# Coder-Yu/QRec

Hardware: NVIDIA H100
Metric: BPR triples/sec at d=64 (higher is better)
Workload: dtype f32

## Files before the change

### qrec_b200/csrc/bpr_kernels.cu

```cuda
#include <cmath>

#include "common.h"
#include "device.cuh"
#include "lane_shape.h"
#include "philox.cuh"
#include "bpr_step.cuh"
#include "um_waves.cuh"

namespace {

using namespace qrec;
using namespace qrec::bpr;

template <typename T, int E>
__global__ void __launch_bounds__(256)
bpr_sgd_ordered_kernel(T* __restrict__ P, T* __restrict__ Q, int d, long long n,
                       const int* __restrict__ u, const int* __restrict__ i,
                       const int* __restrict__ j, const int* __restrict__ wu,
                       const int* __restrict__ wi, const int* __restrict__ wj, int* ver_p,
                       int* ver_q, unsigned long long* ticket, T lr, T reg_u, T reg_i,
                       double* loss) {
  const int lane = threadIdx.x & 31;
  double local_loss = 0.0;
  const T a_u = mul_rn(lr, reg_u), a_i = mul_rn(lr, reg_i);
  while (true) {
    unsigned long long k = 0;
    if (lane == 0) k = atomicAdd(ticket, 1ULL);
    k = __shfl_sync(0xffffffffu, k, 0);
    if (k >= (unsigned long long)n) break;
    const int uu = u[k], ii = i[k], jj = j[k];
    const int* vp = lane == 0 ? ver_p + uu : (lane == 1 ? ver_q + ii : ver_q + jj);
    const int need = lane == 0 ? wu[k] : (lane == 1 ? wi[k] : wj[k]);
    unsigned backoff = 8, polls = 0;
    while (true) {
      const int have = lane < 3 ? ld_acquire_gpu(vp) : need;
      if (__all_sync(0xffffffffu, have == need)) break;
      __nanosleep(backoff);
      if (backoff < 64) backoff <<= 1;
      if (++polls > (1u << 27)) __trap();
    }
    T* pr = P + (size_t)uu * d;
    T* qir = Q + (size_t)ii * d;
    T* qjr = Q + (size_t)jj * d;
    T p[E], qi[E], qj[E];
    T di = 0, dj = 0;
#pragma unroll
    for (int e = 0; e < E; ++e) {
      const int c = e * 32 + lane;
      if (c < d) {
        p[e] = __ldcg(pr + c);
        qi[e] = __ldcg(qir + c);
        qj[e] = __ldcg(qjr + c);
        di += p[e] * qi[e];
        dj += p[e] * qj[e];
      } else {
        p[e] = qi[e] = qj[e] = 0;
      }
    }
    di = warp_sum(di);
    dj = warp_sum(dj);
    const T s = sigmoid_full(sub_rn(di, dj));
    const T g = mul_rn(lr, sub_rn((T)1, s));
#pragma unroll
    for (int e = 0; e < E; ++e) {
      const int c = e * 32 + lane;
      if (c < d) {
        T pn, qin, qjn;
        bpr_update_parity(p[e], qi[e], qj[e], g, a_u, a_i, pn, qin, qjn);
        __stcg(pr + c, pn);
        __stcg(qir + c, qin);
        __stcg(qjr + c, qjn);
      }
    }
    __threadfence();
    __syncwarp();
    if (lane < 3) red_release_gpu_add(const_cast<int*>(vp), 1);
    if (lane == 0) local_loss += neg_log(s);
  }
  if (lane == 0 && local_loss != 0.0) atomicAdd(loss, local_loss);
}

template <int LPR, int VPL, int UNROLL>
__global__ void __launch_bounds__(256)
bpr_sgd_batch_kernel(float* __restrict__ P, float* __restrict__ Q, int nvec, long long n,
                     const int* __restrict__ u, const int* __restrict__ i,
                     const int* __restrict__ j, float lr, float reg_u, float reg_i,
                     double* loss) {
  constexpr int TPW = 32 / LPR;
  const int lane = threadIdx.x & 31;
  const int sub = lane / LPR, l = lane % LPR;
  const long long warp = ((long long)blockIdx.x * blockDim.x + threadIdx.x) >> 5;
  const long long nwarps = ((long long)gridDim.x * blockDim.x) >> 5;
  const int d = nvec * 4;
  const float a_u = lr * reg_u, a_i = lr * reg_i;
  float lsum = 0.f;

  for (long long base = warp * 32; base < n; base += nwarps * 32) {
    const long long k = base + lane;
    int mu = 0, mi = 0, mj = 0;
    if (k < n) {
      mu = __ldg(u + k);
      mi = __ldg(i + k);
      mj = __ldg(j + k);
    }
    const int cnt = (n - base) < 32 ? (int)(n - base) : 32;
    for (int s0 = 0; s0 < cnt; s0 += TPW * UNROLL) {
      float4 p[UNROLL][VPL], qi[UNROLL][VPL], qj[UNROLL][VPL];
      float* pr[UNROLL];
      float* qir[UNROLL];
      float* qjr[UNROLL];
      bool ok[UNROLL];
#pragma unroll
      for (int r = 0; r < UNROLL; ++r) {
        const int t = s0 + r * TPW + sub;
        const int uu = __shfl_sync(0xffffffffu, mu, t & 31);
        const int ii = __shfl_sync(0xffffffffu, mi, t & 31);
        const int jj = __shfl_sync(0xffffffffu, mj, t & 31);
        ok[r] = t < cnt;
        pr[r] = P + (size_t)uu * d + l * 4;
        qir[r] = Q + (size_t)ii * d + l * 4;
        qjr[r] = Q + (size_t)jj * d + l * 4;
#pragma unroll
        for (int v = 0; v < VPL; ++v) {
          if (ok[r] && (l + v * LPR) < nvec) {
            p[r][v] = *reinterpret_cast<const float4*>(pr[r] + v * LPR * 4);
            qi[r][v] = *reinterpret_cast<const float4*>(qir[r] + v * LPR * 4);
            qj[r][v] = *reinterpret_cast<const float4*>(qjr[r] + v * LPR * 4);
          } else {
            p[r][v] = qi[r][v] = qj[r][v] = make_float4(0.f, 0.f, 0.f, 0.f);
          }
        }
      }
#pragma unroll
      for (int r = 0; r < UNROLL; ++r) {
        float x = 0.f;
#pragma unroll
        for (int v = 0; v < VPL; ++v) x += dot4(p[r][v], qi[r][v]) - dot4(p[r][v], qj[r][v]);
        x = group_sum<LPR>(x);
        const float s = fast_sigmoid(x);
        const float g = lr * (1.0f - s);
        if (ok[r]) {
          if (l == 0) lsum += fast_neg_log(s);
#pragma unroll
          for (int v = 0; v < VPL; ++v) {
            if ((l + v * LPR) < nvec) {
              float4 dp, dqi, dqj;
              bpr_step4(p[r][v], qi[r][v], qj[r][v], g, a_u, a_i, dp, dqi, dqj);
              red_add_v4(pr[r] + v * LPR * 4, dp);
              red_add_v4(qir[r] + v * LPR * 4, dqi);
              red_add_v4(qjr[r] + v * LPR * 4, dqj);
            }
          }
        }
      }
    }
  }
  block_add_loss(lsum, loss);
}


template <int LPR>
__global__ void __launch_bounds__(256)
bpr_sgd_staged_kernel(float* __restrict__ P, int nvec, long long n, const int* __restrict__ u,
                      const int* __restrict__ pos_i, const int* __restrict__ pos_j,
                      const float* __restrict__ R, float* __restrict__ D, float lr, float reg_u,
                      float reg_i, double* loss) {
  constexpr int TPW = 32 / LPR;
  const int lane = threadIdx.x & 31;
  const int sub = lane / LPR, l = lane % LPR;
  const long long group = (((long long)blockIdx.x * blockDim.x + threadIdx.x) >> 5) * TPW + sub;
  const long long ngroups = (((long long)gridDim.x * blockDim.x) >> 5) * TPW;
  const int d = nvec * 4;
  const float a_u = lr * reg_u, a_i = lr * reg_i;
  float lsum = 0.f;
  const long long rounds = (n + ngroups - 1) / ngroups;
  for (long long it = 0; it < rounds; ++it) {
    const long long k = it * ngroups + group;
    const bool ok = k < n && l < nvec;
    float4 p = make_float4(0.f, 0.f, 0.f, 0.f), qi = p, qj = p;
    float* pr = nullptr;
    size_t oi = 0, oj = 0;
    if (ok) {
      pr = P + (size_t)__ldg(u + k) * d + l * 4;
      oi = (size_t)__ldg(pos_i + k) * d + l * 4;
      oj = (size_t)__ldg(pos_j + k) * d + l * 4;
      p = *reinterpret_cast<const float4*>(pr);
      qi = __ldg(reinterpret_cast<const float4*>(R + oi));
      qj = __ldg(reinterpret_cast<const float4*>(R + oj));
    }
    float x = dot4(p, qi) - dot4(p, qj);
    x = group_sum<LPR>(x);
    const float s = fast_sigmoid(x);
    const float g = lr * (1.0f - s);
    if (ok) {
      if (l == 0) lsum += fast_neg_log(s);
      float4 dp, dqi, dqj;
      bpr_step4(p, qi, qj, g, a_u, a_i, dp, dqi, dqj);
      red_add_v4(pr, dp);
      *reinterpret_cast<float4*>(D + oi) = dqi;
      *reinterpret_cast<float4*>(D + oj) = dqj;
    }
  }
  block_add_loss(lsum, loss);
}


template <int UNROLL, int TMA_MASK>
__global__ void __launch_bounds__(256)
bpr_sgd_batch_tma_kernel(float* __restrict__ P, float* __restrict__ Q, long long n,
                         const int* __restrict__ u, const int* __restrict__ i,
                         const int* __restrict__ j, float lr, float reg_u, float reg_i,
                         double* loss) {
  constexpr int LPR = 16, TPW = 2, D = 64;
  constexpr int ROWS = ((TMA_MASK >> 0) & 1) + ((TMA_MASK >> 1) & 1) + ((TMA_MASK >> 2) & 1);
  constexpr int SLOT_P = 0, SLOT_I = (TMA_MASK & 1), SLOT_J = (TMA_MASK & 1) + ((TMA_MASK >> 1) & 1);
  constexpr int SLOT_FLOATS = UNROLL * TPW * ROWS * D;
  extern __shared__ __align__(128) float stage[];
  const int lane = threadIdx.x & 31, wib = threadIdx.x >> 5;
  const int sub = lane / LPR, l = lane % LPR;
  const long long warp = ((long long)blockIdx.x * blockDim.x + threadIdx.x) >> 5;
  const long long nwarps = ((long long)gridDim.x * blockDim.x) >> 5;
  const float a_u = lr * reg_u, a_i = lr * reg_i;
  float* my_stage = stage + (size_t)wib * 2 * SLOT_FLOATS;
  float lsum = 0.f;
  int buf = 0;

  for (long long base = warp * 32; base < n; base += nwarps * 32) {
    const long long k = base + lane;
    int mu = 0, mi = 0, mj = 0;
    if (k < n) {
      mu = __ldg(u + k);
      mi = __ldg(i + k);
      mj = __ldg(j + k);
    }
    const int cnt = (n - base) < 32 ? (int)(n - base) : 32;
    for (int s0 = 0; s0 < cnt; s0 += TPW * UNROLL) {
      float4 p[UNROLL], qi[UNROLL], qj[UNROLL];
      int uu[UNROLL], ii[UNROLL], jj[UNROLL];
      bool ok[UNROLL];
#pragma unroll
      for (int r = 0; r < UNROLL; ++r) {
        const int t = s0 + r * TPW + sub;
        uu[r] = __shfl_sync(0xffffffffu, mu, t & 31);
        ii[r] = __shfl_sync(0xffffffffu, mi, t & 31);
        jj[r] = __shfl_sync(0xffffffffu, mj, t & 31);
        ok[r] = t < cnt;
        if (ok[r]) {
          p[r] = *reinterpret_cast<const float4*>(P + (size_t)uu[r] * D + l * 4);
          qi[r] = *reinterpret_cast<const float4*>(Q + (size_t)ii[r] * D + l * 4);
          qj[r] = *reinterpret_cast<const float4*>(Q + (size_t)jj[r] * D + l * 4);
        } else {
          p[r] = qi[r] = qj[r] = make_float4(0.f, 0.f, 0.f, 0.f);
        }
      }
      if (l < 3) asm volatile("cp.async.bulk.wait_group.read 1;" ::: "memory");
      __syncwarp();
      float* slot = my_stage + (size_t)buf * SLOT_FLOATS;
#pragma unroll
      for (int r = 0; r < UNROLL; ++r) {
        float x = dot4(p[r], qi[r]) - dot4(p[r], qj[r]);
        x = group_sum<LPR>(x);
        const float s = fast_sigmoid(x);
        const float g = lr * (1.0f - s);
        if (ok[r]) {
          if (l == 0) lsum += fast_neg_log(s);
          float4 dp, dqi, dqj;
          bpr_step4(p[r], qi[r], qj[r], g, a_u, a_i, dp, dqi, dqj);
          float* trip = slot + (size_t)(r * TPW + sub) * ROWS * D;
          if (TMA_MASK & 1) *reinterpret_cast<float4*>(trip + SLOT_P * D + l * 4) = dp;
          else red_add_v4(P + (size_t)uu[r] * D + l * 4, dp);
          if (TMA_MASK & 2) *reinterpret_cast<float4*>(trip + SLOT_I * D + l * 4) = dqi;
          else red_add_v4(Q + (size_t)ii[r] * D + l * 4, dqi);
          if (TMA_MASK & 4) *reinterpret_cast<float4*>(trip + SLOT_J * D + l * 4) = dqj;
          else red_add_v4(Q + (size_t)jj[r] * D + l * 4, dqj);
        }
      }
      asm volatile("fence.proxy.async.shared::cta;" ::: "memory");
      __syncwarp();
      if (l < 3 && ((TMA_MASK >> l) & 1)) {
        const int srow = (l == 0) ? SLOT_P : (l == 1 ? SLOT_I : SLOT_J);
#pragma unroll
        for (int r = 0; r < UNROLL; ++r) {
          if (ok[r]) {
            float* dst = (l == 0) ? (P + (size_t)uu[r] * D) : (Q + (size_t)(l == 1 ? ii[r] : jj[r]) * D);
            const float* src = slot + (size_t)(r * TPW + sub) * ROWS * D + srow * D;
            asm volatile("cp.reduce.async.bulk.global.shared::cta.bulk_group.add.f32 [%0], [%1], %2;" ::"l"(dst),
                         "r"((uint32_t)__cvta_generic_to_shared(src)), "n"(D * 4)
                         : "memory");
          }
        }
        asm volatile("cp.async.bulk.commit_group;" ::: "memory");
      }
      buf ^= 1;
    }
  }
  if (l < 3) asm volatile("cp.async.bulk.wait_group 0;" ::: "memory");
  block_add_loss(lsum, loss);
}


template <int LPR, int G, bool FULL, bool SAMPLE, int MINB = 3, bool SIG = false>
__global__ void __launch_bounds__(256, MINB)
bpr_sgd_usermajor_kernel(float* __restrict__ P, float* __restrict__ Q, const float* __restrict__ Qr, int nvec, long long n,
                         const int* __restrict__ wave_user, const long long* __restrict__ rowptr,
                         const int* __restrict__ i, const int* __restrict__ j, float lr, float reg_u, float reg_i,
                         double* loss, FusedSampler fs, long long trip_off, const uint32_t* __restrict__ rated_sig) {
  constexpr int GPW = 32 / LPR;
  const int lane = threadIdx.x & 31;
  const int sub = lane / LPR, l = lane % LPR;
  const unsigned gmask = (LPR == 32) ? 0xffffffffu : (((1u << LPR) - 1u) << (sub * LPR));
  const int group = (int)((blockIdx.x * blockDim.x + threadIdx.x) >> 5) * GPW + sub;
  const int ngroups = (int)((gridDim.x * blockDim.x) >> 5) * GPW;
  const int d = FULL ? LPR * 4 : nvec * 4;
  const bool act = FULL ? true : (l < nvec);
  const float a_u = lr * reg_u, a_i = lr * reg_i;
  const float one_m_au = 1.0f - a_u, one_m_ai = 1.0f - a_i;
  float lsum = 0.f;
  qrec::pdl_launch_dependents();
  bool waited = false;
  const int ub = __ldg(wave_user + 1);
  for (int uu = __ldg(wave_user) + group; uu < ub; uu += ngroups) {
    long long lo = __ldg(rowptr + uu) - trip_off, hi = __ldg(rowptr + uu + 1) - trip_off;
    lo = lo > 0 ? lo : 0;
    hi = hi < n ? hi : n;
    if (lo >= hi) continue;
    float* prow = P + (size_t)uu * d + l * 4;
    float4 p = act ? *reinterpret_cast<const float4*>(prow) : make_float4(0.f, 0.f, 0.f, 0.f);
    long long rated_lo = 0, rated_hi = 0;
    if (SAMPLE) {
      rated_lo = __ldg(fs.rated_rowptr + uu);
      rated_hi = __ldg(fs.rated_rowptr + uu + 1);
    }
    for (long long base = lo; base < hi; base += LPR) {
      const int m = (hi - base) < LPR ? (int)(hi - base) : LPR;
      int mj = 0, mi = 0;
      if (l < m) {
        mi = __ldg(i + base + l);
        if (SAMPLE) {
          if (SIG)
            mj = qrec::sample_negative_sig(base + l + trip_off, fs.epoch, fs.seed_lo, fs.seed_hi, fs.num_items,
                                           fs.rated_cols, rated_lo, rated_hi,
                                           rated_sig + (size_t)uu * qrec::RATED_SIG_WORDS);
          else
            mj = qrec::sample_negative(base + l + trip_off, fs.epoch, fs.seed_lo, fs.seed_hi, fs.num_items, fs.rated_cols,
                                       rated_lo, rated_hi);
        } else {
          mj = __ldg(j + base + l);
        }
      }
      if (!waited) {
        qrec::pdl_wait();
        waited = true;
      }
      if (SAMPLE && l < m && fs.j_out != nullptr) fs.j_out[base + l] = mj;
      for (int t0 = 0; t0 < m; t0 += G) {
        float4 qi[G], qj[G];
        int ri[G], rj[G];
#pragma unroll
        for (int f = 0; f < G; ++f) {
          ri[f] = __shfl_sync(gmask, mi, sub * LPR + ((t0 + f) & (LPR - 1)));
          rj[f] = __shfl_sync(gmask, mj, sub * LPR + ((t0 + f) & (LPR - 1)));
          if (t0 + f < m && act) {
            qi[f] = qrec::ldg_no_l1_v4(reinterpret_cast<const float4*>(Qr + (size_t)ri[f] * d + l * 4));
            qj[f] = qrec::ldg_no_l1_v4(reinterpret_cast<const float4*>(Qr + (size_t)rj[f] * d + l * 4));
          } else {
            qi[f] = qj[f] = make_float4(0.f, 0.f, 0.f, 0.f);
          }
        }
#pragma unroll
        for (int f = 0; f < G; ++f) {
          if (t0 + f < m) {
            float x = dot4(p, qi[f]) - dot4(p, qj[f]);
            x = group_sum<LPR>(x, gmask);
            const float s = fast_sigmoid(x);
            const float g = lr * (1.0f - s);
            if (l == 0) lsum += fast_neg_log(s);
            if (act) {
              float4 dqi, dqj;
              bpr_step4_inplace(p, qi[f], qj[f], g, one_m_au, g * one_m_ai, a_i, dqi, dqj);
              red_add_v4(Q + (size_t)ri[f] * d + l * 4, dqi);
              red_add_v4(Q + (size_t)rj[f] * d + l * 4, dqj);
            }
          }
        }
      }
    }
    if (act) {
      const float4 p0 = __ldcg(reinterpret_cast<const float4*>(prow));
      red_add_v4(prow, make_float4(p.x - p0.x, p.y - p0.y, p.z - p0.z, p.w - p0.w));
    }
  }
  if (!waited) qrec::pdl_wait();
  block_add_loss(lsum, loss);
}

using UserMajorKernel = decltype(&bpr_sgd_usermajor_kernel<16, 4, true, false>);

template <int LPR>
UserMajorKernel usermajor_kernel(int nvec, bool sample, bool sig) {
  if (nvec != LPR)
    return sample ? bpr_sgd_usermajor_kernel<LPR, 4, false, true> : bpr_sgd_usermajor_kernel<LPR, 4, false, false>;
  if (sig) return bpr_sgd_usermajor_kernel<LPR, 2, true, true, 4, true>;
  return sample ? bpr_sgd_usermajor_kernel<LPR, 2, true, true, 4> : bpr_sgd_usermajor_kernel<LPR, 4, true, false>;
}

constexpr int UM_SNAPSHOT_THREADS = 512, UM_SNAPSHOT_CTAS_PER_SM = 4;
__global__ void __launch_bounds__(UM_SNAPSHOT_THREADS, UM_SNAPSHOT_CTAS_PER_SM)
um_snapshot_kernel(const float4* __restrict__ Q, float4* __restrict__ Qr, long long n4) {
  const unsigned long long keep = qrec::l2_policy_evict_last();
  qrec::pdl_wait();
  qrec::pdl_launch_dependents();
  const long long stride = (long long)gridDim.x * blockDim.x;
  long long k = (long long)blockIdx.x * blockDim.x + threadIdx.x;
  for (; k + 3 * stride < n4; k += 4 * stride) {
    float4 v[4];
#pragma unroll
    for (int r = 0; r < 4; ++r) v[r] = qrec::ld_stream_v4(Q + k + r * stride, keep);
#pragma unroll
    for (int r = 0; r < 4; ++r) qrec::st_hint_v4(Qr + k + r * stride, v[r], keep);
  }
  for (; k < n4; k += stride) qrec::st_hint_v4(Qr + k, qrec::ld_stream_v4(Q + k, keep), keep);
}

__global__ void __launch_bounds__(256)
um_wave_table_kernel(const long long* __restrict__ rowptr, int n_users, long long n, long long trip_off,
                     long long wave_chunks, long long nwaves, int* __restrict__ wave_user) {
  const long long w = (long long)blockIdx.x * blockDim.x + threadIdx.x;
  if (w <= nwaves) wave_user[w] = um_wave_first_user(rowptr, n_users, n, trip_off, wave_chunks, w);
}

__global__ void __launch_bounds__(256)
rated_signature_kernel(int n_users, const long long* __restrict__ rowptr, const int* __restrict__ cols,
                       uint32_t* __restrict__ sig) {
  const int lane = threadIdx.x & 31;
  const long long warp = ((long long)blockIdx.x * blockDim.x + threadIdx.x) >> 5;
  const long long nwarps = ((long long)gridDim.x * blockDim.x) >> 5;
  for (long long uu = warp; uu < n_users; uu += nwarps) {
    const long long lo = __ldg(rowptr + uu), hi = __ldg(rowptr + uu + 1);
    for (long long e = lo + lane; e < hi; e += 32) {
      const int c = __ldg(cols + e);
      atomicOr(sig + (size_t)uu * qrec::RATED_SIG_WORDS + ((c >> 5) & (qrec::RATED_SIG_WORDS - 1)), 1u << (c & 31));
    }
  }
}

template <typename T>
__global__ void __launch_bounds__(256)
sumsq_kernel(const T* __restrict__ x, long long n, double* out) {
  double acc = 0.0;
  const long long tid = (long long)blockIdx.x * blockDim.x + threadIdx.x;
  const long long stride = (long long)gridDim.x * blockDim.x;
  if constexpr (sizeof(T) == 4) {
    const long long n4 = n >> 2;
    const float4* x4 = reinterpret_cast<const float4*>(x);
    for (long long k = tid; k < n4; k += stride) {
      const float4 v = __ldg(x4 + k);
      acc += (double)v.x * v.x + (double)v.y * v.y + (double)v.z * v.z + (double)v.w * v.w;
    }
    for (long long k = (n4 << 2) + tid; k < n; k += stride) acc += (double)x[k] * x[k];
  } else {
    for (long long k = tid; k < n; k += stride) acc += (double)x[k] * (double)x[k];
  }
  acc = warp_sum(acc);
  __shared__ double wsum[8];
  if ((threadIdx.x & 31) == 0) wsum[threadIdx.x >> 5] = acc;
  __syncthreads();
  if (threadIdx.x == 0) {
    double t = 0.0;
    for (int w = 0; w < (int)(blockDim.x >> 5); ++w) t += wsum[w];
    atomicAdd(out, t);
  }
}

template <typename T>
int launch_ordered(T* P, T* Q, int d, long long n, const int* u, const int* i, const int* j,
                   const int* wu, const int* wi, const int* wj, int* ver_p, int* ver_q,
                   unsigned long long* ticket, T lr, T reg_u, T reg_i, double* loss,
                   int n_warps, cudaStream_t st) {
  QREC_REQUIRE(P && Q && loss && ticket && ver_p && ver_q, "bpr_sgd_ordered: null pointer");
  QREC_REQUIRE(d >= 1 && d <= 256, "bpr_sgd_ordered: d=%d unsupported (1..256)", d);
  QREC_REQUIRE(n >= 0, "bpr_sgd_ordered: n < 0");
  if (n == 0) return QREC_OK;
  QREC_REQUIRE(u && i && j && wu && wi && wj, "bpr_sgd_ordered: null index pointer");
  const int grid = n_warps > 0 ? capped_grid((n_warps + 7) / 8, 2) : sm_count() * 2;
  with_lane_elems(d, [&](auto e) {
    bpr_sgd_ordered_kernel<T, decltype(e)::E><<<grid, 256, 0, st>>>(P, Q, d, n, u, i, j, wu, wi, wj, ver_p, ver_q,
                                                                    ticket, lr, reg_u, reg_i, loss);
  });
  QREC_LAUNCH_CHECK();
  return QREC_OK;
}

}

namespace qrec {
int launch_bpr_batch(float* P, float* Q, int d, long long n, const int* u, const int* i,
                     const int* j, float lr, float reg_u, float reg_i, double* loss,
                     cudaStream_t st) {
  QREC_REQUIRE(P && Q && loss, "bpr_sgd_batch: null pointer");
  QREC_REQUIRE(d >= 4 && d <= 256 && (d % 4) == 0, "bpr_sgd_batch: d=%d unsupported (multiple of 4, 4..256)", d);
  QREC_REQUIRE(n >= 0, "bpr_sgd_batch: n < 0");
  if (n == 0) return QREC_OK;
  QREC_REQUIRE(u && i && j, "bpr_sgd_batch: null index pointer");
  const int nvec = d / 4;
  const long long warps_needed = (n + 31) / 32;
  const int grid = capped_grid((warps_needed + 7) / 8, 8);
  with_row_shape<256>(nvec, [&](auto s) {
    using S = decltype(s);
    bpr_sgd_batch_kernel<S::LPR, S::VPL, S::UNROLL><<<grid, 256, 0, st>>>(P, Q, nvec, n, u, i, j, lr, reg_u, reg_i,
                                                                          loss);
  });
  QREC_LAUNCH_CHECK();
  return QREC_OK;
}
}

extern "C" {

int qrec_bpr_sgd_ordered_f32(float* P, float* Q, int32_t d, int64_t n, const int32_t* u,
                             const int32_t* i, const int32_t* j, const int32_t* wu,
                             const int32_t* wi, const int32_t* wj, int32_t* ver_p,
                             int32_t* ver_q, unsigned long long* ticket, float lr, float reg_u,
                             float reg_i, double* loss, int32_t n_warps, void* stream) {
  return launch_ordered<float>(P, Q, d, n, u, i, j, wu, wi, wj, ver_p, ver_q, ticket, lr, reg_u,
                               reg_i, loss, n_warps, (cudaStream_t)stream);
}

int qrec_bpr_sgd_ordered_f64(double* P, double* Q, int32_t d, int64_t n, const int32_t* u,
                             const int32_t* i, const int32_t* j, const int32_t* wu,
                             const int32_t* wi, const int32_t* wj, int32_t* ver_p,
                             int32_t* ver_q, unsigned long long* ticket, double lr,
                             double reg_u, double reg_i, double* loss, int32_t n_warps, void* stream) {
  return launch_ordered<double>(P, Q, d, n, u, i, j, wu, wi, wj, ver_p, ver_q, ticket, lr, reg_u,
                                reg_i, loss, n_warps, (cudaStream_t)stream);
}

int qrec_bpr_sgd_batch_f32(float* P, float* Q, int32_t d, int64_t n, const int32_t* u,
                           const int32_t* i, const int32_t* j, float lr, float reg_u,
                           float reg_i, double* loss, void* stream) {
  return qrec::launch_bpr_batch(P, Q, d, n, u, i, j, lr, reg_u, reg_i, loss, (cudaStream_t)stream);
}

int qrec_bpr_sgd_batch_tma_f32(float* P, float* Q, int32_t d, int64_t n, const int32_t* u,
                               const int32_t* i, const int32_t* j, float lr, float reg_u,
                               float reg_i, double* loss, void* stream) {
  QREC_REQUIRE(P && Q && loss, "qrec_bpr_sgd_batch_tma_f32: null pointer");
  QREC_REQUIRE(d == 64, "qrec_bpr_sgd_batch_tma_f32: only d=64 (got %d); use qrec_bpr_sgd_batch_f32", d);
  QREC_REQUIRE(n >= 0, "qrec_bpr_sgd_batch_tma_f32: n < 0");
  if (n == 0) return QREC_OK;
  QREC_REQUIRE(u && i && j, "qrec_bpr_sgd_batch_tma_f32: null index pointer");
  constexpr int UN = 4, MASK = 1;
  constexpr int smem = 8 * 2 * UN * 2 * 64 * 4;
  QREC_CUDA(allow_dynamic_smem((const void*)bpr_sgd_batch_tma_kernel<UN, MASK>, smem));
  const int grid = capped_grid(((n + 31) / 32 + 7) / 8, 2);
  bpr_sgd_batch_tma_kernel<UN, MASK><<<grid, 256, smem, (cudaStream_t)stream>>>(P, Q, n, u, i, j, lr, reg_u, reg_i, loss);
  QREC_LAUNCH_CHECK();
  return QREC_OK;
}

}

namespace qrec {
int launch_usermajor(float* P, float* Q, int32_t d, int32_t n_users, int64_t n, const int64_t* rowptr,
                     const int32_t* i, const int32_t* j, float lr, float reg_u, float reg_i, double* loss,
                     bool sample, const int64_t* rated_rowptr, const int32_t* rated_cols, int32_t num_items,
                     uint64_t seed, uint32_t epoch, int32_t* j_out, long long trip_off, cudaStream_t st,
                     const uint32_t* rated_sig) {
  if (n <= 0) return QREC_OK;
  QREC_REQUIRE(num_items >= 1, "qrec user-major epoch: num_items=%d (the item table's rows) must be given", num_items);
  FusedSampler fs = {reinterpret_cast<const long long*>(rated_rowptr), rated_cols, num_items, (uint32_t)seed,
                     (uint32_t)(seed >> 32), epoch, j_out};
  const int nvec = d / 4;
  const int lpr = row_lpr(nvec);
  const bool sig = sample && rated_sig != nullptr;
  const UserMajorKernel kernel =
      with_row_shape<128>(nvec, [&](auto s) { return usermajor_kernel<decltype(s)::LPR>(nvec, sample, sig); });
  int occ = 3;
  if (cudaOccupancyMaxActiveBlocksPerMultiprocessor(&occ, kernel, 256, 0) != cudaSuccess || occ < 1) occ = 3;
  const long long per_block = 8 * (32 / lpr);
  const long long max_users = n < n_users ? n : n_users;
  const int grid = capped_grid((max_users + per_block - 1) / per_block, occ);
  const size_t q_bytes = (size_t)num_items * d * sizeof(float);
  const long long wave = um_wave_chunks(n, num_items, d);
  const long long nwaves = um_num_waves(n, wave);
  float* Qr = nullptr;
  int* wave_user = nullptr;
  QREC_CUDA(cudaMallocAsync(reinterpret_cast<void**>(&Qr), q_bytes, st));
  const int rc = [&]() -> int {
    QREC_CUDA(cudaMallocAsync(reinterpret_cast<void**>(&wave_user), sizeof(int) * (size_t)(nwaves + 1), st));
    um_wave_table_kernel<<<(unsigned)((nwaves + 256) / 256), 256, 0, st>>>(reinterpret_cast<const long long*>(rowptr), n_users,
                                                                          n, trip_off, wave, nwaves, wave_user);
    QREC_CUDA(cudaGetLastError());
    count_launch();
    cudaLaunchAttribute pdl;
    pdl.id = cudaLaunchAttributeProgrammaticStreamSerialization;
    pdl.val.programmaticStreamSerializationAllowed = 1;
    const auto launch = [&](auto* fn, dim3 g, dim3 b, bool chained, auto... args) {
      cudaLaunchConfig_t cfg = {};
      cfg.gridDim = g;
      cfg.blockDim = b;
      cfg.stream = st;
      cfg.attrs = chained ? &pdl : nullptr;
      cfg.numAttrs = chained ? 1 : 0;
      return cudaLaunchKernelEx(&cfg, fn, args...);
    };
    const long long n4 = (long long)(q_bytes / sizeof(float4));
    const int copy_grid = sm_count() * UM_SNAPSHOT_CTAS_PER_SM;
    for (long long w = 0; w < nwaves; ++w) {
      QREC_CUDA(launch(um_snapshot_kernel, dim3(copy_grid), dim3(UM_SNAPSHOT_THREADS), w > 0,
                       reinterpret_cast<const float4*>(Q), reinterpret_cast<float4*>(Qr), n4));
      count_launch();
      QREC_CUDA(launch(kernel, dim3(grid), dim3(256), true, P, Q, static_cast<const float*>(Qr), nvec,
                       (long long)n, static_cast<const int*>(wave_user + w), reinterpret_cast<const long long*>(rowptr), i, j,
                       lr, reg_u, reg_i, loss, fs, trip_off, rated_sig));
      if (w + 1 < nwaves) count_launch();
    }
    return QREC_OK;
  }();
  if (wave_user != nullptr) QREC_CUDA(cudaFreeAsync(wave_user, st));
  QREC_CUDA(cudaFreeAsync(Qr, st));
  if (rc != QREC_OK) return rc;
  QREC_LAUNCH_CHECK();
  return QREC_OK;
}
}

extern "C" {

int qrec_bpr_sgd_usermajor_f32(float* P, float* Q, int32_t d, int32_t n_users, int64_t n, int32_t num_items,
                               const int64_t* rowptr, const int32_t* i, const int32_t* j, float lr, float reg_u, float reg_i,
                               double* loss, void* stream) {
  QREC_REQUIRE(P && Q && loss, "qrec_bpr_sgd_usermajor_f32: null pointer");
  QREC_REQUIRE(d >= 4 && d <= 128 && (d % 4) == 0, "qrec_bpr_sgd_usermajor_f32: d=%d unsupported (multiple of 4, 4..128)", d);
  QREC_REQUIRE(n_users >= 0 && n >= 0, "qrec_bpr_sgd_usermajor_f32: negative size");
  if (n_users == 0 || n == 0) return QREC_OK;
  QREC_REQUIRE(rowptr && i && j, "qrec_bpr_sgd_usermajor_f32: null index pointer");
  return qrec::launch_usermajor(P, Q, d, n_users, n, rowptr, i, j, lr, reg_u, reg_i, loss, false, nullptr, nullptr, num_items,
                                0, 0, nullptr, 0, (cudaStream_t)stream, nullptr);
}

int qrec_bpr_epoch_usermajor_f32(float* P, float* Q, int32_t d, int32_t n_users, int64_t n, const int64_t* rowptr,
                                 const int32_t* i, const int64_t* rated_rowptr, const int32_t* rated_cols,
                                 int32_t num_items, uint64_t seed, uint32_t epoch, int32_t* j_out, float lr,
                                 float reg_u, float reg_i, double* loss, void* stream) {
  QREC_REQUIRE(P && Q && loss, "qrec_bpr_epoch_usermajor_f32: null pointer");
  QREC_REQUIRE(d >= 4 && d <= 128 && (d % 4) == 0, "qrec_bpr_epoch_usermajor_f32: d=%d unsupported (multiple of 4, 4..128)", d);
  QREC_REQUIRE(n_users >= 0 && n >= 0 && num_items >= 1, "qrec_bpr_epoch_usermajor_f32: bad size");
  if (n_users == 0 || n == 0) return QREC_OK;
  QREC_REQUIRE(rowptr && i && rated_rowptr && rated_cols, "qrec_bpr_epoch_usermajor_f32: null index pointer");
  return qrec::launch_usermajor(P, Q, d, n_users, n, rowptr, i, nullptr, lr, reg_u, reg_i, loss, true, rated_rowptr,
                                rated_cols, num_items, seed, epoch, j_out, 0, (cudaStream_t)stream, nullptr);
}

int qrec_rated_signature_build(int32_t n_users, const int64_t* rated_rowptr, const int32_t* rated_cols,
                               uint32_t* sig, void* stream) {
  QREC_REQUIRE(n_users >= 0, "qrec_rated_signature_build: n_users < 0");
  if (n_users == 0) return QREC_OK;
  QREC_REQUIRE(rated_rowptr && rated_cols && sig, "qrec_rated_signature_build: null pointer");
  cudaStream_t st = (cudaStream_t)stream;
  QREC_CUDA(cudaMemsetAsync(sig, 0, (size_t)n_users * qrec::RATED_SIG_WORDS * sizeof(uint32_t), st));
  rated_signature_kernel<<<capped_grid(((long long)n_users + 7) / 8, 8), 256, 0, st>>>(n_users, reinterpret_cast<const long long*>(rated_rowptr),
                                                     rated_cols, sig);
  QREC_LAUNCH_CHECK();
  return QREC_OK;
}

int qrec_bpr_epoch_usermajor_sig_f32(float* P, float* Q, int32_t d, int32_t n_users, int64_t n, const int64_t* rowptr,
                                     const int32_t* i, const int64_t* rated_rowptr, const int32_t* rated_cols,
                                     const uint32_t* rated_sig, int32_t num_items, uint64_t seed, uint32_t epoch,
                                     int32_t* j_out, float lr, float reg_u, float reg_i, double* loss, void* stream) {
  QREC_REQUIRE(P && Q && loss, "qrec_bpr_epoch_usermajor_sig_f32: null pointer");
  QREC_REQUIRE(d == 16 || d == 32 || d == 64 || d == 128,
               "qrec_bpr_epoch_usermajor_sig_f32: d=%d unsupported (16, 32, 64 or 128); use qrec_bpr_epoch_usermajor_f32", d);
  QREC_REQUIRE(n_users >= 0 && n >= 0 && num_items >= 1, "qrec_bpr_epoch_usermajor_sig_f32: bad size");
  if (n_users == 0 || n == 0) return QREC_OK;
  QREC_REQUIRE(rowptr && i && rated_rowptr && rated_cols && rated_sig, "qrec_bpr_epoch_usermajor_sig_f32: null index pointer");
  return qrec::launch_usermajor(P, Q, d, n_users, n, rowptr, i, nullptr, lr, reg_u, reg_i, loss, true, rated_rowptr,
                                rated_cols, num_items, seed, epoch, j_out, 0, (cudaStream_t)stream, rated_sig);
}

int qrec_bpr_sgd_staged_f32(float* P, int32_t d, int64_t n, const int32_t* u, const int32_t* pos_i,
                            const int32_t* pos_j, const float* R, float* D, float lr, float reg_u,
                            float reg_i, double* loss, void* stream) {
  QREC_REQUIRE(d >= 4 && d <= 128 && (d % 4) == 0, "qrec_bpr_sgd_staged_f32: d=%d unsupported (multiple of 4, 4..128)", d);
  QREC_REQUIRE(n >= 0, "qrec_bpr_sgd_staged_f32: n < 0");
  if (n == 0) return QREC_OK;
  QREC_REQUIRE(P && u && pos_i && pos_j && R && D && loss, "qrec_bpr_sgd_staged_f32: null pointer");
  const int nvec = d / 4;
  cudaStream_t st = (cudaStream_t)stream;
  with_row_shape<128>(nvec, [&](auto s) {
    constexpr int LPR = decltype(s)::LPR;
    const long long per_block = 8 * (32 / LPR);
    const int grid = capped_grid((n + per_block - 1) / per_block, 8);
    bpr_sgd_staged_kernel<LPR><<<grid, 256, 0, st>>>(P, nvec, n, u, pos_i, pos_j, R, D, lr, reg_u, reg_i, loss);
  });
  QREC_LAUNCH_CHECK();
  return QREC_OK;
}

int qrec_sumsq_f32(const float* x, int64_t n, double* out, void* stream) {
  QREC_REQUIRE(out && (x || n == 0) && n >= 0, "qrec_sumsq_f32: bad argument");
  if (n == 0) return QREC_OK;
  QREC_REQUIRE((reinterpret_cast<uintptr_t>(x) & 15) == 0, "qrec_sumsq_f32: x not 16-byte aligned");
  sumsq_kernel<float><<<capped_grid((n / 4 + 255) / 256 + 1, 8), 256, 0, (cudaStream_t)stream>>>(x, n, out);
  QREC_LAUNCH_CHECK();
  return QREC_OK;
}

int qrec_table_snapshot_f32(const float* src, float* dst, int64_t n, void* stream) {
  QREC_REQUIRE(n >= 0 && (n % 4) == 0, "qrec_table_snapshot_f32: n=%lld must be a multiple of 4", (long long)n);
  if (n == 0) return QREC_OK;
  QREC_REQUIRE(src && dst, "qrec_table_snapshot_f32: null pointer");
  QREC_REQUIRE(((reinterpret_cast<uintptr_t>(src) | reinterpret_cast<uintptr_t>(dst)) & 15) == 0,
               "qrec_table_snapshot_f32: src and dst must be 16-byte aligned");
  um_snapshot_kernel<<<sm_count() * UM_SNAPSHOT_CTAS_PER_SM, UM_SNAPSHOT_THREADS, 0, (cudaStream_t)stream>>>(reinterpret_cast<const float4*>(src),
                                                                                 reinterpret_cast<float4*>(dst), n / 4);
  QREC_LAUNCH_CHECK();
  return QREC_OK;
}

int qrec_sumsq_f64(const double* x, int64_t n, double* out, void* stream) {
  QREC_REQUIRE(out && (x || n == 0) && n >= 0, "qrec_sumsq_f64: bad argument");
  if (n == 0) return QREC_OK;
  sumsq_kernel<double><<<capped_grid((n + 255) / 256, 8), 256, 0, (cudaStream_t)stream>>>(x, n, out);
  QREC_LAUNCH_CHECK();
  return QREC_OK;
}

}
```

### qrec_b200/csrc/philox.cuh

```cuda
#pragma once
#include <cstdint>

namespace qrec {

__device__ __forceinline__ void philox4x32_10(uint32_t c0, uint32_t c1, uint32_t c2, uint32_t c3,
                                              uint32_t k0, uint32_t k1, uint32_t out[4]) {
  constexpr uint32_t M0 = 0xD2511F53u, M1 = 0xCD9E8D57u, W0 = 0x9E3779B9u, W1 = 0xBB67AE85u;
#pragma unroll
  for (int r = 0; r < 10; ++r) {
    const uint32_t hi0 = __umulhi(M0, c0), lo0 = M0 * c0;
    const uint32_t hi1 = __umulhi(M1, c2), lo1 = M1 * c2;
    const uint32_t n0 = hi1 ^ c1 ^ k0, n1 = lo1, n2 = hi0 ^ c3 ^ k1, n3 = lo0;
    c0 = n0; c1 = n1; c2 = n2; c3 = n3;
    k0 += W0; k1 += W1;
  }
  out[0] = c0; out[1] = c1; out[2] = c2; out[3] = c3;
}

__device__ __forceinline__ int sample_negative(long long k, uint32_t epoch, uint32_t seed_lo, uint32_t seed_hi,
                                               int num_items, const int* __restrict__ cols, long long lo0,
                                               long long hi0) {
  const bool saturated = (hi0 - lo0) >= (long long)num_items;
  uint32_t attempt = 0;
  while (true) {
    uint32_t w[4];
    philox4x32_10((uint32_t)k, (uint32_t)((unsigned long long)k >> 32), attempt, epoch, seed_lo, seed_hi, w);
    const int j = (int)(((unsigned long long)w[0] * (unsigned long long)(uint32_t)num_items) >> 32);
    if (saturated) return j;
    long long lo = lo0, hi = hi0;
    bool hit = false;
    while (lo < hi) {
      const long long mid = (lo + hi) >> 1;
      const int c = __ldg(cols + mid);
      if (c < j) lo = mid + 1;
      else if (c > j) hi = mid;
      else { hit = true; break; }
    }
    if (!hit) return j;
    ++attempt;
  }
}

constexpr int RATED_SIG_WORDS = 16;
__device__ __forceinline__ int sample_negative_sig(long long k, uint32_t epoch, uint32_t seed_lo, uint32_t seed_hi,
                                                   int num_items, const int* __restrict__ cols, long long lo0,
                                                   long long hi0, const uint32_t* __restrict__ sig) {
  const bool saturated = (hi0 - lo0) >= (long long)num_items;
  uint32_t attempt = 0;
  while (true) {
    uint32_t w[4];
    philox4x32_10((uint32_t)k, (uint32_t)((unsigned long long)k >> 32), attempt, epoch, seed_lo, seed_hi, w);
    const int j = (int)(((unsigned long long)w[0] * (unsigned long long)(uint32_t)num_items) >> 32);
    if (saturated) return j;
    const uint32_t word = __ldg(sig + ((j >> 5) & (RATED_SIG_WORDS - 1)));
    if (((word >> (j & 31)) & 1u) == 0u) return j;
    long long lo = lo0, hi = hi0;
    bool hit = false;
    while (lo < hi) {
      const long long mid = (lo + hi) >> 1;
      const int c = __ldg(cols + mid);
      if (c < j) lo = mid + 1;
      else if (c > j) hi = mid;
      else { hit = true; break; }
    }
    if (!hit) return j;
    ++attempt;
  }
}

struct FusedSampler {
  const long long* rated_rowptr;
  const int* rated_cols;
  int num_items;
  uint32_t seed_lo, seed_hi, epoch;
  int* j_out;
};

}
```

Before: 3.217 billion.

## Stage rated items and positive indices in shared memory for user-major BPR

For short rated rows (up to 64 items), each user's rated item list is copied into per-group shared memory. Negative sampling then does a linear scan over 16-byte words instead of a global binary search or signature lookup. Positive item indices are also staged in shared memory in chunks, replacing the per-triple shuffle. The final P row update changes from an atomic delta-add to a plain store, which assumes each user row is owned by a single group. The change adds shared memory use that may lower occupancy, plus instrumentation macros that compile to nothing by default.

New measurement: 3.257 billion, median of 6. +1.3%, better.

```diff
diff --git a/qrec_b200/csrc/bpr_kernels.cu b/qrec_b200/csrc/bpr_kernels.cu
--- a/qrec_b200/csrc/bpr_kernels.cu
+++ b/qrec_b200/csrc/bpr_kernels.cu
@@ -6,6 +6,14 @@
 #include "philox.cuh"
 #include "bpr_step.cuh"
 #include "um_waves.cuh"
+
+#ifndef QREC_K1_MARK_PROLOGUE
+#define QREC_K1_MARK_PROLOGUE(user)
+#define QREC_K1_MARK_FIRST_GATHER(user, first)
+#define QREC_K1_MARK_LAST_RED(user, wave_first_user)
+#define QREC_UM_COPY_MARK_START()
+#define QREC_UM_COPY_MARK_END()
+#endif
 
 namespace {
 
@@ -318,6 +326,10 @@
   float lsum = 0.f;
   qrec::pdl_launch_dependents();
   bool waited = false;
+  constexpr int RCAP = qrec::RATED_STAGE_CAP;
+  __shared__ __align__(16) int stage[8 * GPW][SAMPLE ? 2 * RCAP : RCAP];
+  int* const pos = stage[(threadIdx.x >> 5) * GPW + sub];
+  int* const rated = pos + RCAP;
   const int ub = __ldg(wave_user + 1);
   for (int uu = __ldg(wave_user) + group; uu < ub; uu += ngroups) {
     long long lo = __ldg(rowptr + uu) - trip_off, hi = __ldg(rowptr + uu + 1) - trip_off;
@@ -326,39 +338,56 @@
     if (lo >= hi) continue;
     float* prow = P + (size_t)uu * d + l * 4;
     float4 p = act ? *reinterpret_cast<const float4*>(prow) : make_float4(0.f, 0.f, 0.f, 0.f);
-    long long rated_lo = 0, rated_hi = 0;
+    const int* rcols = nullptr;
+    int nr = 0;
+    bool staged = false;
+    __syncwarp(gmask);
     if (SAMPLE) {
-      rated_lo = __ldg(fs.rated_rowptr + uu);
-      rated_hi = __ldg(fs.rated_rowptr + uu + 1);
-    }
-    for (long long base = lo; base < hi; base += LPR) {
-      const int m = (hi - base) < LPR ? (int)(hi - base) : LPR;
-      int mj = 0, mi = 0;
+      const long long rated_lo = __ldg(fs.rated_rowptr + uu);
+      rcols = fs.rated_cols + rated_lo;
+      nr = (int)(__ldg(fs.rated_rowptr + uu + 1) - rated_lo);
+      staged = nr <= RCAP && nr < fs.num_items;
+      if (staged)
+        for (int t = l; t < ((nr + 3) & ~3); t += LPR) rated[t] = t < nr ? __ldg(rcols + t) : -1;
+    }
+    const int cnt = (int)(hi - lo);
+    for (int b0 = 0; b0 < cnt; b0 += LPR) {
+      const long long base = lo + b0;
+      const int b = b0 & (RCAP - 1);
+      if (b == 0) {
+        if (b0 != 0) __syncwarp(gmask);
+        const int ms = (cnt - b0) < RCAP ? cnt - b0 : RCAP;
+        for (int t = l; t < ms; t += LPR) pos[t] = __ldg(i + base + t);
+        __syncwarp(gmask);
+      }
+      const int m = (cnt - b0) < LPR ? cnt - b0 : LPR;
+      int mj = 0;
       if (l < m) {
-        mi = __ldg(i + base + l);
         if (SAMPLE) {
-          if (SIG)
-            mj = qrec::sample_negative_sig(base + l + trip_off, fs.epoch, fs.seed_lo, fs.seed_hi, fs.num_items,
-                                           fs.rated_cols, rated_lo, rated_hi,
+          if (staged)
+            mj = qrec::sample_negative_staged(base + l + trip_off, fs.epoch, fs.seed_lo, fs.seed_hi, fs.num_items, rated, nr);
+          else if (SIG)
+            mj = qrec::sample_negative_sig(base + l + trip_off, fs.epoch, fs.seed_lo, fs.seed_hi, fs.num_items, rcols, 0, nr,
                                            rated_sig + (size_t)uu * qrec::RATED_SIG_WORDS);
           else
-            mj = qrec::sample_negative(base + l + trip_off, fs.epoch, fs.seed_lo, fs.seed_hi, fs.num_items, fs.rated_cols,
-                                       rated_lo, rated_hi);
+            mj = qrec::sample_negative(base + l + trip_off, fs.epoch, fs.seed_lo, fs.seed_hi, fs.num_items, rcols, 0, nr);
         } else {
           mj = __ldg(j + base + l);
         }
       }
       if (!waited) {
+        QREC_K1_MARK_PROLOGUE(uu);
         qrec::pdl_wait();
         waited = true;
       }
       if (SAMPLE && l < m && fs.j_out != nullptr) fs.j_out[base + l] = mj;
+      QREC_K1_MARK_FIRST_GATHER(uu, b0 == 0);
       for (int t0 = 0; t0 < m; t0 += G) {
         float4 qi[G], qj[G];
         int ri[G], rj[G];
 #pragma unroll
         for (int f = 0; f < G; ++f) {
-          ri[f] = __shfl_sync(gmask, mi, sub * LPR + ((t0 + f) & (LPR - 1)));
+          ri[f] = pos[(b + t0 + f) & (RCAP - 1)];
           rj[f] = __shfl_sync(gmask, mj, sub * LPR + ((t0 + f) & (LPR - 1)));
           if (t0 + f < m && act) {
             qi[f] = qrec::ldg_no_l1_v4(reinterpret_cast<const float4*>(Qr + (size_t)ri[f] * d + l * 4));
@@ -385,10 +414,8 @@
         }
       }
     }
-    if (act) {
-      const float4 p0 = __ldcg(reinterpret_cast<const float4*>(prow));
-      red_add_v4(prow, make_float4(p.x - p0.x, p.y - p0.y, p.z - p0.z, p.w - p0.w));
-    }
+    if (act) *reinterpret_cast<float4*>(prow) = p;
+    QREC_K1_MARK_LAST_RED(uu, __ldg(wave_user));
   }
   if (!waited) qrec::pdl_wait();
   block_add_loss(lsum, loss);
@@ -410,6 +437,7 @@
   const unsigned long long keep = qrec::l2_policy_evict_last();
   qrec::pdl_wait();
   qrec::pdl_launch_dependents();
+  QREC_UM_COPY_MARK_START();
   const long long stride = (long long)gridDim.x * blockDim.x;
   long long k = (long long)blockIdx.x * blockDim.x + threadIdx.x;
   for (; k + 3 * stride < n4; k += 4 * stride) {
@@ -420,6 +448,7 @@
     for (int r = 0; r < 4; ++r) qrec::st_hint_v4(Qr + k + r * stride, v[r], keep);
   }
   for (; k < n4; k += stride) qrec::st_hint_v4(Qr + k, qrec::ld_stream_v4(Q + k, keep), keep);
+  QREC_UM_COPY_MARK_END();
 }
 
 __global__ void __launch_bounds__(256)
diff --git a/qrec_b200/csrc/philox.cuh b/qrec_b200/csrc/philox.cuh
--- a/qrec_b200/csrc/philox.cuh
+++ b/qrec_b200/csrc/philox.cuh
@@ -68,6 +68,29 @@
   }
 }
 
+constexpr int RATED_STAGE_CAP = 64;
+struct alignas(16) StagedWord { int x, y, z, w; };
+__device__ __forceinline__ bool staged_row_contains(const int* s, int n, int j) {
+  bool hit = false;
+#pragma unroll 2
+  for (int t = 0; t < n; t += 4) {
+    const StagedWord v = *reinterpret_cast<const StagedWord*>(s + t);
+    hit |= (v.x == j) | (v.y == j) | (v.z == j) | (v.w == j);
+  }
+  return hit;
+}
+__device__ __forceinline__ int sample_negative_staged(long long k, uint32_t epoch, uint32_t seed_lo, uint32_t seed_hi,
+                                                      int num_items, const int* s, int n) {
+  uint32_t attempt = 0;
+  while (true) {
+    uint32_t w[4];
+    philox4x32_10((uint32_t)k, (uint32_t)((unsigned long long)k >> 32), attempt, epoch, seed_lo, seed_hi, w);
+    const int j = (int)(((unsigned long long)w[0] * (unsigned long long)(uint32_t)num_items) >> 32);
+    if (!staged_row_contains(s, n, j)) return j;
+    ++attempt;
+  }
+}
+
 struct FusedSampler {
   const long long* rated_rowptr;
   const int* rated_cols;
```
